# xuanjiangliu/robotic-discovery-platform

Hardware: AMD Instinct MI355X
Metric: U-Net train imgs/sec at 256×256 (1/2/4/8 GPU); e2e frames/sec + p50 latency (higher is better)
Workload: dtype bf16; 1 GPU; model=UNet(3,1) bilinear decoder, 17.26M params, global_batch=64, per_gpu_batch=64, image_size=256, parallelism=dp1, impl=native, optimizer=Adam(lr=1e-4), loss=bce, sync_bn=False, hipgraph=False

## Files before the change

### csrc/bindings.cpp

```cpp
#include <torch/extension.h>
#include <c10/hip/HIPGuard.h>
#include <c10/hip/HIPStream.h>
#include <hip/hip_runtime.h>
#include <dlfcn.h>
#include <link.h>
#include <chrono>
#include <cmath>
#include <climits>
#include <cstdlib>
#include <cstring>
#include <functional>
#include <memory>
#include <vector>
#include <array>

#include "rdp_api.h"

namespace {

hipStream_t cur_stream() { return c10::hip::getCurrentHIPStream().stream(); }

void note_device(int& dev, const torch::Tensor& t) {
  if (!t.defined() || !t.is_cuda()) return;
  const int d = t.get_device();
// ... 461 lines not shown
    if (sp) TORCH_CHECK(rows + conv_stats_rows((long)nn * a1.H * a1.W, Cout, bm_pref) <= avail_rows, "stats slab too small");
    RdpConv c;
    conv_bind(c, kX1, a1, n0, nn);
    conv_bind(c, kX2, a2, n0, nn);
    conv_bind(c, kY1, o1, n0, nn);
    conv_bind(c, kY2, o2, n0, nn);
    conv_weights(c, w);
    c.stats = sp ? sp + (long)rows * 2 * Cout : nullptr;
    c.Cout = Cout;
    c.escale = esc; c.eshift = esh; c.erelu = relu;
    RdpConvFuse fuse;
    if (pool) { fuse.pool = po.image(n0); fuse.ppitch = po.pitch; }
    if (up) {
      fuse.up = uo.image(n0); fuse.upitch = uo.pitch; fuse.uH = uo.H; fuse.uW = uo.W;
      fuse.uoy = up_oy; fuse.uox = up_ox;
    }
    float* const wsp = ws ? ws->data_ptr<float>() : nullptr;
    const long wsn = ws ? (long)ws->numel() : 0L;
    const bool want_fused = pool || up;
    auto pooled = std::make_shared<int>(0);
    const int fmode = wfrag && esc && !sp && !y2 && taps == 9 && !packed && bm_pref == 0
                          ? rdp_conv_rowband_frag_auto(nn, a1.H, a1.W, a1.C, c.C2, Cout) : 0;
    int r = -1;
    if (fmode > 0) {
      RdpConv cf = c;
      cf.w = wfrag->data_ptr(); cf.wbytes = wfrag->numel() * 2; cf.ldw = 0;
      const long pbytes = pool ? po.span_bytes(nn) : 0;
      const int rb = RDP_PLAN(rdp_conv_rowband_ex(cf, fuse.pool, pbytes, fuse.ppitch, fmode, st));
      if (rb >= 0) {
        *pooled = rb == 1 ? 1 : 0;
        r = 0;
      }
    }
    if (r < 0) {
      r = RDP_PLAN(rdp_conv_igemm(c, taps, packed, bm_pref, wsp, wsn, fuse, want_fused ? pooled.get() : nullptr,
                                  RdpConvBnBwd{}, nullptr, st));
    }
    TORCH_CHECK(r >= 0, "conv_fwd: unsupported shape (C1=", a1.C, ", C2=", c.C2, ", Cout=", Cout, ")");
    void* const py1 = c.y1;
    const int oH = o1.H, oW = o1.W, oC = o1.C, op1 = o1.pitch;
    if (pool && !*pooled)
      TORCH_CHECK(RDP_PLAN(rdp_maxpool2_fwd(py1, op1, fuse.pool, fuse.ppitch, nn, oH, oW, oC, st)) == 0,
                  "conv_fwd: maxpool");
    if (up && !*pooled)
      TORCH_CHECK(RDP_PLAN(rdp_upsample2_fwd(py1, op1, fuse.up, fuse.upitch, nn, oH, oW, fuse.uH, fuse.uW, fuse.uoy,
                                             fuse.uox, oC, nullptr, st)) == 0,
                  "conv_fwd: upsample");
    rows += r;
  }
  return rows;
}


int conv_wgrad(torch::Tensor x1, c10::optional<torch::Tensor> x2, torch::Tensor dy, int taps, int packed, int cin_real,
               torch::Tensor slab, torch::Tensor out, int accumulate, int splits, int variant) {
  Act a1 = act(x1, "x1"), a2;
  if (x2) a2 = act(*x2, "x2");
  Act d = act(dy, "dy");
  TORCH_CHECK(d.N == a1.N && d.H == a1.H && d.W == a1.W, "dy spatial mismatch");
  check_f32(slab, "slab");
  check_f32(out, "out");
  const int Cin = packed ? cin_real : a1.C + (x2 ? a2.C : 0);
  TORCH_CHECK(out.numel() == (long)d.C * taps * Cin, "wgrad out numel mismatch");
  const int nc = chunk_images({a1, a2, d}, a1.N);
  int r = 0;
  for (int n0 = 0; n0 < a1.N; n0 += nc) {
    const int nn = std::min(nc, a1.N - n0);
    void* const px1 = a1.image(n0);
    void* const px2 = x2 ? a2.image(n0) : nullptr;
    void* const pdy = d.image(n0);
    const long bx1 = a1.span_bytes(nn), bx2 = x2 ? a2.span_bytes(nn) : 0, bdy = d.span_bytes(nn);
    const int C2 = x2 ? a2.C : 0, p2 = x2 ? a2.pitch : 0, acc = n0 > 0 ? 1 : accumulate;
    float* const slp = slab.data_ptr<float>();
    const long sln = slab.numel();
    float* const outp = out.data_ptr<float>();
    r = RDP_PLAN(rdp_conv_wgrad(px1, px2, bx1, bx2, a1.C, C2, a1.pitch, p2, pdy, bdy, d.pitch, slp, sln, outp, acc, nn,
                                a1.H, a1.W, d.C, taps, packed, cin_real, splits, variant, st));
    TORCH_CHECK(r >= 0, "conv_wgrad: unsupported shape or slab too small (code ", r, ")");
  }
  return r;
}

int wgrad_first_bn(torch::Tensor x, torch::Tensor da, torch::Tensor y, torch::Tensor coef, torch::Tensor coef2,
                   torch::Tensor slab, torch::Tensor out, int cin_real, int accumulate, int splits) {
  Act a = act(x, "x"), d = act(da, "da"), b = act(y, "y");
  TORCH_CHECK(a.C == 8 && d.C == 64 && b.C == 64, "wgrad_first_bn: x must have 8 (packed) and da / y 64 channels");
  TORCH_CHECK(d.N == a.N && d.H == a.H && d.W == a.W && b.N == a.N && b.H == a.H && b.W == a.W,
              "wgrad_first_bn: spatial mismatch");
  check_f32(coef, "coef"); check_f32(coef2, "coef2"); check_f32(slab, "slab"); check_f32(out, "out");
  TORCH_CHECK(coef.numel() >= 4 * 64 && coef2.numel() >= 3 * 64, "wgrad_first_bn: coef / coef2 too small");
  TORCH_CHECK(out.numel() == 64l * 9 * cin_real, "wgrad_first_bn: out numel mismatch");
  if (a.bytes >= (1l << 31) || d.bytes >= (1l << 31) || b.bytes >= (1l << 31)) return -1;
  if (((long)a.N * a.H * a.W) % 64) return -1;
  const int r = RDP_PLAN(rdp_wgrad_first_bn(a.ptr, a.bytes, a.pitch, d.ptr, d.bytes, d.pitch, b.ptr, b.bytes, b.pitch,
                                            coef.data_ptr<float>(), coef2.data_ptr<float>(), slab.data_ptr<float>(),
                                            slab.numel(), out.data_ptr<float>(), accumulate, a.N, a.H, a.W, cin_real,
                                            splits, st));
  TORCH_CHECK(r > 0, "wgrad_first_bn: slab too small (code ", r, ")");
  return r;
}

long wgrad_slab_elems(int N, int H, int W, int Cin, int Cout, int taps, int packed, int splits) {
  return rdp_conv_wgrad_slab_elems(N, H, W, Cin, Cout, taps, packed, splits);
}

void bn_finalize(torch::Tensor stats, int T, long count, torch::Tensor gamma, torch::Tensor beta,
                 c10::optional<torch::Tensor> rmean, c10::optional<torch::Tensor> rvar,
                 c10::optional<torch::Tensor> nbt, double momentum, double eps, torch::Tensor coef,
                 c10::optional<torch::Tensor> ws) {
  const int C = gamma.numel();
  check_f32(stats, "stats"); check_f32(gamma, "gamma"); check_f32(beta, "beta"); check_f32(coef, "coef");
  TORCH_CHECK(stats.numel() >= (long)T * 2 * C && coef.numel() >= 4 * C, "bn_finalize sizes");
  float* rm = nullptr; float* rv = nullptr; long long* nb = nullptr;
  if (rmean) { check_f32(*rmean, "rmean"); rm = rmean->data_ptr<float>(); }
  if (rvar) { check_f32(*rvar, "rvar"); rv = rvar->data_ptr<float>(); }
  if (nbt) { TORCH_CHECK(nbt->scalar_type() == torch::kInt64 && nbt->is_cuda(), "nbt int64"); nb = (long long*)nbt->data_ptr(); }
  RDP_PLAN(rdp_bn_finalize(stats.data_ptr<float>(), T, C, count, gamma.data_ptr<float>(), beta.data_ptr<float>(), rm, rv, nb,
                  (float)momentum, (float)eps, coef.data_ptr<float>(), ws_ptr(ws, 2 * C), st));
}

void bn_eval_coef(torch::Tensor gamma, torch::Tensor beta, torch::Tensor rmean, torch::Tensor rvar, double eps,
                  torch::Tensor coef) {
  const int C = gamma.numel();
  check_f32(coef, "coef");
  RDP_PLAN(rdp_bn_eval_coef(C, gamma.data_ptr<float>(), beta.data_ptr<float>(), rmean.data_ptr<float>(), rvar.data_ptr<float>(),
                   (float)eps, coef.data_ptr<float>(), st));
}

void bn_relu_apply(torch::Tensor y, torch::Tensor out, torch::Tensor coef, int relu) {
  Act a = act(y, "y"), o = act(out, "out");
  TORCH_CHECK(a.N == o.N && a.H == o.H && a.W == o.W && a.C == o.C, "bn_relu_apply shape");
  TORCH_CHECK(coef.numel() >= 4 * a.C, "coef");
  TORCH_CHECK(RDP_PLAN(rdp_bn_relu_apply(a.ptr, a.pitch, o.ptr, o.pitch, coef.data_ptr<float>(), a.N * a.H * a.W, a.C, relu,
                                st)) == 0, "bn_relu_apply");
}

int conv_dgrad_bnred(torch::Tensor dy, torch::Tensor w, torch::Tensor dx, torch::Tensor y_bn, torch::Tensor coef,
                     torch::Tensor partial) {
  Act a = act(dy, "dy"), o = act(dx, "dx"), b = act(y_bn, "y_bn");
  check_w(w);
  TORCH_CHECK(o.N == a.N && o.H == a.H && o.W == a.W && b.N == a.N && b.H == a.H && b.W == a.W && b.C == o.C,
              "conv_dgrad_bnred: shape mismatch");
  TORCH_CHECK(w.size(0) == o.C, "w rows != Cout");
  check_f32(coef, "coef");
  check_f32(partial, "partial");
  TORCH_CHECK(coef.numel() >= 4l * o.C, "coef must hold 4*C floats");
  TORCH_CHECK(partial.numel() >= 1024l * 2 * o.C, "partial too small");
  if (chunk_images({a, o, b}, a.N) < a.N) return -1;
  RdpConv c;
  conv_bind(c, kX1, a, 0, a.N);
  conv_bind(c, kY1, o, 0, a.N);
  conv_weights(c, w);
  c.Cout = o.C;
  c.stats = partial.data_ptr<float>();
  RdpRingFuse f;
  f.bn_y = b.ptr; f.bn_ypitch = b.pitch; f.bn_coef = coef.data_ptr<float>();
  return RDP_PLAN(rdp_conv_ring_ex(c, 256, f, st));
}

int conv_dgrad_splitk_bnred(torch::Tensor dy, torch::Tensor w, torch::Tensor dx, torch::Tensor y_bn,
                            torch::Tensor coef, torch::Tensor partial, c10::optional<torch::Tensor> ws) {
  Act a = act(dy, "dy"), o = act(dx, "dx"), b = act(y_bn, "y_bn");
  check_w(w);
  TORCH_CHECK(o.N == a.N && o.H == a.H && o.W == a.W && b.N == a.N && b.H == a.H && b.W == a.W && b.C == o.C,
              "conv_dgrad_splitk_bnred: shape mismatch");
  TORCH_CHECK(w.size(0) == o.C && w.size(1) >= 9l * a.C, "conv_dgrad_splitk_bnred: w must be [Cout][9 * Cin]");
  check_f32(coef, "coef");
  check_f32(partial, "partial");
  TORCH_CHECK(coef.numel() >= 4l * o.C, "coef must hold 4*C floats");
  TORCH_CHECK(partial.numel() >= 512l * 2 * o.C, "partial too small");
  if (ws) check_f32(*ws, "ws");
  if (chunk_images({a, o, b}, a.N) < a.N) return -1;
  RdpConv c;
  conv_bind(c, kX1, a, 0, a.N);
  conv_bind(c, kY1, o, 0, a.N);
  conv_weights(c, w);
  c.Cout = o.C;
  RdpConvBnBwd bn;
  bn.bny = b.ptr; bn.bnypitch = b.pitch; bn.bncoef = coef.data_ptr<float>(); bn.bnpart = partial.data_ptr<float>();
  float* const wsp = ws ? ws->data_ptr<float>() : nullptr;
// ... 1078 lines not shown
              "u8 / int16 HxW contiguous CPU tensor");
  const int h = img.size(0), w = img.size(1), bpp = (int)img.element_size();
  TORCH_CHECK(h > 0 && w > 0 && level >= 0 && level <= 9 && bands >= 1, "png_encode: bad size / level / bands");
  std::string out((size_t)rdp_png_encode_bound(w, h, bpp, bands), '\0');
  long len;
  {
    py::gil_scoped_release nogil;
    len = rdp_png_encode_gray((const uint8_t*)img.data_ptr(), w, h, bpp, level, bands, (uint8_t*)&out[0],
                              (long)out.size());
  }
  TORCH_CHECK(len > 0, "png encode failed");
  out.resize((size_t)len);
  return py::bytes(out);
}


void preprocess(torch::Tensor bgr, torch::Tensor ystart, torch::Tensor ysize, torch::Tensor yw, torch::Tensor xstart,
                torch::Tensor xsize, torch::Tensor xw, torch::Tensor out, int rgb) {
  TORCH_CHECK(bgr.is_cuda() && bgr.scalar_type() == torch::kUInt8 && bgr.dim() == 3 && bgr.size(2) == 3 &&
              bgr.is_contiguous(), "bgr u8 HxWx3");
  Act o = act(out, "out");
  TORCH_CHECK(o.N == 1 && o.C == 8 && o.pitch == 8, "out must be [1,OH,OW,8] contiguous");
  TORCH_CHECK(ystart.numel() == o.H && xstart.numel() == o.W && yw.numel() == (long)o.H * 16 &&
              xw.numel() == (long)o.W * 16, "aa tables");
  rdp_preprocess(bgr.data_ptr(), bgr.size(0), bgr.size(1), ystart.data_ptr<int>(), ysize.data_ptr<int>(),
                 yw.data_ptr<float>(), xstart.data_ptr<int>(), xsize.data_ptr<int>(), xw.data_ptr<float>(), o.H, o.W,
                 rgb, o.ptr, unplanned_stream());
}

void mask_upsample(torch::Tensor m, torch::Tensor out, torch::Tensor count) {
  TORCH_CHECK(m.is_cuda() && m.scalar_type() == torch::kUInt8 && m.dim() == 2 && m.is_contiguous(), "m");
  TORCH_CHECK(out.is_cuda() && out.scalar_type() == torch::kUInt8 && out.dim() == 2 && out.is_contiguous(), "out");
  TORCH_CHECK(count.is_cuda() && count.scalar_type() == torch::kInt32, "count int32");
  rdp_mask_upsample(m.data_ptr(), m.size(0), m.size(1), out.data_ptr(), out.size(0), out.size(1),
                    (unsigned*)count.data_ptr(), unplanned_stream());
}

}

void register_serve_runtime(py::module_& m);

PYBIND11_MODULE(TORCH_EXTENSION_NAME, m) {
  register_serve_runtime(m);
  m.doc() = "rdp MI355X (gfx950) HIP kernels";
  m.def("stream_wait", &stream_wait, "waiter stream waits for the work issued so far on waitee (recorded in plans)");
  m.def("event_create", &event_create, "runtime-owned cross-stream event (id)");
  m.def("event_record", &event_record, py::arg("id"), py::arg("stream"), "record event id on stream (recorded in plans)");
  m.def("stream_wait_event", &stream_wait_event, py::arg("stream"), py::arg("id"),
        "stream waits for the last record of event id (recorded in plans)");
  m.def("plan_begin", &plan_begin);
  m.def("plan_end", &plan_end);
  m.def("plan_abort", &plan_abort);
  m.def("plan_replay", &plan_replay, py::arg("id"), py::arg("host_call") = py::none());
  m.def("plan_kinds", &plan_kinds);
  m.def("plan_recording", &plan_recording);
  m.def("comm_bind", &comm_bind, "resolve RCCL from the library torch loaded; returns its path");
  m.def("comm_all_reduce", on_device(&comm_all_reduce), py::arg("buf"), py::arg("comm"),
        "in-place SUM all-reduce over an RCCL communicator on the current stream (recorded in plans)");
  m.def("rows_fold", on_device(&rows_fold), py::arg("buf"), py::arg("rows"), py::arg("width"), py::arg("out"));
  m.def("rows_hilo", on_device(&rows_hilo), py::arg("sums"), py::arg("buf"), py::arg("width"));
  m.def("comm_async_error", &comm_async_error, py::arg("comm"), "(code, message) of ncclCommGetAsyncError");
  m.def("comm_abort", &comm_abort, py::arg("comm"), "ncclCommAbort");
  m.def("comm_info", &comm_info, py::arg("comm"), "(ncclCommCount, ncclCommUserRank, ncclCommCuDevice)");
  m.def("comm_emulate", &comm_emulate, py::arg("us"), py::arg("blocks"), py::arg("scratch") = py::none(),
        py::arg("traffic_bytes") = 0, "RDP_DDP_EMULATE: the modelled all-reduce on the current stream (recorded in plans)");
  m.def("plan_mark", &plan_mark, "record a host call point (replay calls host_call(tag) there)");
  m.def("plan_pause", &plan_pause);
  m.def("plan_resume", &plan_resume);
  m.def("plan_size", &plan_size);
  m.def("plan_free", &plan_free);
  m.def("conv_fwd", on_device(&conv_fwd), py::arg("x1"), py::arg("x2"), py::arg("w"), py::arg("taps"), py::arg("packed"),
        py::arg("y1"), py::arg("y2"), py::arg("stats"), py::arg("bm_pref"), py::arg("affine"), py::arg("relu"),
        py::arg("ws") = py::none(), py::arg("pool") = py::none(), py::arg("up") = py::none(),
        py::arg("up_oy") = 0, py::arg("up_ox") = 0, py::arg("wfrag") = py::none());
  m.def("conv_ws_elems", [](int N, int H, int W, int C1, int C2, int Cout, int taps, int packed, int bm_pref) {
    return rdp_conv_ws_elems(N, H, W, C1, C2, Cout, taps, packed, bm_pref);
  });
  m.def("conv_stats_rows", &conv_stats_rows);
  m.def("conv_wgrad", on_device(&conv_wgrad), py::arg("x1"), py::arg("x2"), py::arg("dy"), py::arg("taps"),
        py::arg("packed"), py::arg("cin_real"), py::arg("slab"), py::arg("out"), py::arg("accumulate"),
        py::arg("splits"), py::arg("variant"));
  m.def("conv_fwd_bnin", on_device(&conv_fwd_bnin), py::arg("x_pre"), py::arg("w"), py::arg("y"), py::arg("stats"),
        py::arg("in_coef"), py::arg("a_out") = py::none());
  m.def("wgrad_first_bn", on_device(&wgrad_first_bn));
  m.def("wgrad_slab_elems", &wgrad_slab_elems);
  m.def("wgrad_halo_slab_elems", &rdp_conv_wgrad_halo_slab_elems);
  m.def("bn_finalize", on_device(&bn_finalize));
  m.def("bn_eval_coef", on_device(&bn_eval_coef));
  m.def("bn_relu_apply", on_device(&bn_relu_apply));
  m.def("bn_relu_bwd_reduce", on_device(&bn_relu_bwd_reduce));
  m.def("conv_dgrad_bnred", on_device(&conv_dgrad_bnred));
  m.def("conv_dgrad_splitk_bnred", on_device(&conv_dgrad_splitk_bnred), py::arg("dy"), py::arg("w"), py::arg("dx"),
        py::arg("y_bn"), py::arg("coef"), py::arg("partial"), py::arg("ws") = py::none());
  m.def("bn_bwd_finalize", on_device(&bn_bwd_finalize));
  m.def("bn_relu_bwd_apply", on_device(&bn_relu_bwd_apply));
  m.def("maxpool2_fwd", on_device(&maxpool2_fwd));
  m.def("maxpool2_bwd", on_device(&maxpool2_bwd));
  m.def("bn_relu_apply_pool", on_device(&bn_relu_apply_pool));
  m.def("maxpool2_bwd_bn_reduce", on_device(&maxpool2_bwd_bn_reduce));
  m.def("upsample2_fwd", on_device(&upsample2_fwd), py::arg("x"), py::arg("out"), py::arg("oy"), py::arg("ox"),
        py::arg("coef") = py::none());
  m.def("upT_shuffle", on_device(&upT_shuffle));
  m.def("conv_upT_fwd", on_device(&conv_upT_fwd));
  m.def("conv_upT_dgrad", on_device(&conv_upT_dgrad));
  m.def("conv_wgrad_upT", on_device(&conv_wgrad_upT));
  m.def("upT_unshuffle", on_device(&upT_unshuffle));
  m.def("colsum_bf16", on_device(&colsum_bf16));
  m.def("upsample2_bwd", on_device(&upsample2_bwd), py::arg("dout"), py::arg("dx"), py::arg("oy"), py::arg("ox"),
        py::arg("y") = py::none(), py::arg("coef") = py::none(), py::arg("partial") = py::none());
  m.def("head_partial_blocks", &head_partial_blocks);
  m.def("head_fwd", on_device(&head_fwd), py::arg("a"), py::arg("w"), py::arg("b"), py::arg("target"), py::arg("logits"),
        py::arg("partial"), py::arg("sums"), py::arg("loss"), py::arg("dice_w"), py::arg("dice_eps"),
        py::arg("coef") = py::none(), py::arg("gpart") = py::none(), py::arg("bnpart") = py::none(),
        py::arg("gscale") = 1.0);
  m.def("head_grad_finalize", on_device(&head_grad_finalize));
  m.def("head_bwd", on_device(&head_bwd), py::arg("a"), py::arg("w"), py::arg("logits"), py::arg("target"), py::arg("sums"),
        py::arg("da"), py::arg("partial"), py::arg("gw"), py::arg("gb"), py::arg("dice_w"), py::arg("dice_eps"),
        py::arg("gscale"), py::arg("coef") = py::none(), py::arg("bnpart") = py::none());
  m.def("head_bn_bwd_apply", on_device(&head_bn_bwd_apply));
  m.def("head_mask", on_device(&head_mask));
  m.def("headk_partial_blocks", &headk_partial_blocks);
  m.def("headk_fwd", on_device(&headk_fwd), py::arg("a"), py::arg("w"), py::arg("b"), py::arg("labels"),
        py::arg("logits"), py::arg("partial"), py::arg("sums"), py::arg("loss"), py::arg("class_weights") = py::none(),
        py::arg("dice_w") = 0.0, py::arg("dice_eps") = 1.0);
  m.def("headk_bwd", on_device(&headk_bwd), py::arg("a"), py::arg("w"), py::arg("logits"), py::arg("labels"),
        py::arg("sums"), py::arg("da"), py::arg("partial"), py::arg("gw"), py::arg("gb"), py::arg("gscale") = 1.0,
        py::arg("class_weights") = py::none(), py::arg("dice_w") = 0.0, py::arg("dice_eps") = 1.0);
  m.def("headk_mask", on_device(&headk_mask), py::arg("a"), py::arg("w"), py::arg("b"), py::arg("cls"),
        py::arg("mask"));
  m.def("seg_confusion_blocks", &seg_confusion_blocks);
  m.def("seg_confusion_block_pixels", &seg_confusion_block_pixels);
  m.def("seg_confusion", on_device(&seg_confusion), py::arg("logits"), py::arg("target"), py::arg("K"),
        py::arg("counts"), py::arg("thr") = 0.0, py::arg("max_blocks") = 0);
  m.def("conv_head_mask", on_device(&conv_head_mask));
  m.def("conv_headk_mask", on_device(&conv_headk_mask), py::arg("x"), py::arg("w"), py::arg("coef"), py::arg("head_w"),
        py::arg("head_b"), py::arg("cls"), py::arg("mask"));
  m.def("conv_rowband_chain", on_device(&conv_rowband_chain));
  m.def("conv_rowband", on_device(&conv_rowband));
  m.def("rowband_frag_mode", &rdp_conv_rowband_frag_auto, py::arg("n"), py::arg("h"), py::arg("w"), py::arg("c1"),
        py::arg("c2"), py::arg("cout"));
  m.def("adam", on_device(&adam), py::arg("p"), py::arg("g"), py::arg("m"), py::arg("v"), py::arg("shadow"), py::arg("lr"),
        py::arg("b1"), py::arg("b2"), py::arg("eps"), py::arg("wd"), py::arg("gscale"), py::arg("step"),
        py::arg("inc") = true, py::arg("max_blocks") = 0);
  m.def("grad_sqnorm_blocks", &grad_sqnorm_blocks, py::arg("n"));
  m.def("grad_sqnorm", on_device(&grad_sqnorm), py::arg("g"), py::arg("partial"), py::arg("max_blocks") = 0);
  m.def("optim_ctl", on_device(&optim_ctl), py::arg("partial"), py::arg("nblocks"), py::arg("gscale"), py::arg("clip"),
        py::arg("sched"), py::arg("warmup"), py::arg("total"), py::arg("min_ratio"), py::arg("step"), py::arg("ctl"));
  m.def("adam_ctl", on_device(&adam_ctl), py::arg("p"), py::arg("g"), py::arg("m"), py::arg("v"), py::arg("shadow"),
        py::arg("lr"), py::arg("b1"), py::arg("b2"), py::arg("eps"), py::arg("wd"), py::arg("gscale"), py::arg("step"),
        py::arg("ctl"), py::arg("inc") = true, py::arg("max_blocks") = 0);
  m.def("cast_bf16", on_device(&cast_bf16));
  m.def("h2d_copy", &h2d_copy, py::arg("src"), py::arg("dst"));
  m.def("wprep", on_device(&wprep), py::arg("master"), py::arg("out"), py::arg("segs"), py::arg("nseg"),
        py::arg("step") = py::none(), py::arg("blocks") = 0);
  m.def("wseg_size", &rdp_wseg_size);
  m.def("parcur", &parcur);
  m.def("batch_preprocess", on_device(&batch_preprocess));
  m.def("geo_frames_batch", on_device(&geo_frames_batch));
  m.def("geo_edges", on_device(&geo_edges), py::arg("mask"), py::arg("depth"), py::arg("fx"), py::arg("fy"), py::arg("cx"),
        py::arg("cy"), py::arg("scale"), py::arg("work_i"), py::arg("work_d"), py::arg("pts"), py::arg("npts"),
        py::arg("out"), py::arg("kout"), py::arg("nbins"), py::arg("top"), py::arg("min_points"),
        py::arg("edges") = py::none(), py::arg("hdr") = py::none(), py::arg("m256") = py::none(),
        py::arg("cov") = py::none(), py::arg("sorted") = py::none(), py::arg("gperm") = py::none(),
        py::arg("mask_host") = py::none());
  m.def("geo_nblocks", &geo_nblocks);
  m.def("geo_spline", on_device(&geo_spline), py::arg("out"), py::arg("kout"), py::arg("npts"), py::arg("sorted"),
        py::arg("gperm"), py::arg("u"), py::arg("res"), py::arg("s"), py::arg("k"), py::arg("nsamp"), py::arg("eps"),
// ... 28 lines not shown
```

### csrc/conv_wgrad.hip

```cpp
#include "common.h"
#include "rdp_api.h"
#include <algorithm>
#include <stdlib.h>
#include <string.h>

struct WgradArgs {
  const u16* x1;
  const u16* x2;
  uint32_t xbytes1, xbytes2;
  int C1, C2, pitch1, pitch2;
  const u16* dy;
  uint32_t dybytes;
  int dypitch;
  float* slab;
  int H, W, M, Cout, Cin;
  int taps, packed;
  int ncols, ncols_pad;
  int colTiles, coutTiles, splits;
  int pix_per_split;
  uint32_t fw_m, fw_s, fh_m, fh_s;
  int uH2 = 0, uW2 = 0, uoy = 0, uox = 0;
};

RDP_DEV int swz(int p) { return (((p >> 1) & 1) << 1) | (((p >> 3) & 1) << 2); }
// ... 650 lines not shown
      else hipLaunchKernelGGL((conv_wgrad_halo_kernel<64, false>), dim3(nblk), dim3(256), 0, s, h);
    }
    rdp_wgrad_reduce(slab, out, h.splits, Cout, h.ncols, 9, a.Cin, a.Cin, accumulate, s);
    return h.splits;
  }
  a.colTiles = (a.ncols + 255) / 256;
  a.ncols_pad = a.colTiles * 256;
  a.coutTiles = Cout / 64;
  if (splits < 1) splits = 1;
  int pps = (a.M + splits - 1) / splits;
  pps = (pps + 63) / 64 * 64;
  a.pix_per_split = pps;
  a.splits = (a.M + pps - 1) / pps;
  if ((long)a.splits * Cout * a.ncols_pad > slab_elems) return -2;
  if ((long)a.splits * Cout * a.ncols_pad * 4l >= (1l << 31)) return -3;
  FastDiv fw = make_fastdiv(W), fh = make_fastdiv(H);
  a.fw_m = fw.m; a.fw_s = fw.s; a.fh_m = fh.m; a.fh_s = fh.s;
  const int nblk = a.colTiles * a.coutTiles * a.splits;
  if (packed) hipLaunchKernelGGL((conv_wgrad_kernel<true>), dim3(nblk), dim3(512), 0, s, a);
  else hipLaunchKernelGGL((conv_wgrad_kernel<false>), dim3(nblk), dim3(512), 0, s, a);
  rdp_wgrad_reduce(slab, out, a.splits, Cout, a.ncols_pad, taps, packed ? 8 : a.Cin, packed ? cin_real : a.Cin,
                   accumulate, s);
  return a.splits;
}

extern "C" int rdp_conv_wgrad_upT(const void* du, long dubytes, int C, int dupitch, int H2, int W2, int oy, int ox,
                                  const void* x, long xbytes, int Cin, int xpitch, int N, int h, int w, float* slab,
                                  long slab_elems, float* out, int accumulate, int splits, hipStream_t s) {
  if (C % 64 || Cin % 64 || oy < 0 || ox < 0 || 2 * h + oy > H2 || 2 * w + ox > W2) return -1;
  if (dubytes >= (1l << 31) || xbytes >= (1l << 31)) return -1;
  WgradArgs a;
  a.x1 = (const u16*)du; a.x2 = nullptr; a.xbytes1 = (uint32_t)dubytes; a.xbytes2 = 0;
  a.C1 = C; a.C2 = 0; a.pitch1 = dupitch; a.pitch2 = dupitch;
  a.dy = (const u16*)x; a.dybytes = (uint32_t)xbytes; a.dypitch = xpitch;
  a.slab = slab; a.H = h; a.W = w; a.M = N * h * w; a.Cout = Cin;
  a.taps = 4; a.packed = 0; a.Cin = C; a.ncols = 4 * C;
  a.uH2 = H2; a.uW2 = W2; a.uoy = oy; a.uox = ox;
  a.colTiles = (a.ncols + 255) / 256;
  a.ncols_pad = a.colTiles * 256;
  a.coutTiles = Cin / 64;
  if (splits < 1) splits = 1;
  int pps = (a.M + splits - 1) / splits;
  pps = (pps + 63) / 64 * 64;
  a.pix_per_split = pps;
  a.splits = (a.M + pps - 1) / pps;
  if ((long)a.splits * a.Cout * a.ncols_pad > slab_elems) return -2;
  if ((long)a.splits * a.Cout * a.ncols_pad * 4l >= (1l << 31)) return -3;
  FastDiv fw = make_fastdiv(w), fh = make_fastdiv(h);
  a.fw_m = fw.m; a.fw_s = fw.s; a.fh_m = fh.m; a.fh_s = fh.s;
  const int nblk = a.colTiles * a.coutTiles * a.splits;
  hipLaunchKernelGGL((conv_wgrad_kernel<false, true>), dim3(nblk), dim3(512), 0, s, a);
  rdp_wgrad_reduce(slab, out, a.splits, Cin, a.ncols_pad, 4, C, C, accumulate, s);
  return a.splits;
}

struct FirstWgradArgs {
  const u16* x;
  uint32_t xbytes;
  int xpitch;
  const u16* da;
  uint32_t dabytes;
  int dapitch;
  const u16* y;
  uint32_t ybytes;
  int ypitch;
  const float* coef;
  const float* coef2;
  float* slab;
  uint32_t slab_bytes;
  int H, W, M, pix_per_split;
  uint32_t fw_m, fw_s, fh_m, fh_s;
};
constexpr int FWG_NCOLS = 80;

RDP_DEV void fw_unpack8(const uint4& v, float* f) {
  const uint32_t w[4] = {v.x, v.y, v.z, v.w};
#pragma unroll
  for (int i = 0; i < 4; ++i) {
    f[2 * i] = __uint_as_float(w[i] << 16);
    f[2 * i + 1] = __uint_as_float(w[i] & 0xffff0000u);
  }
}

__global__ __launch_bounds__(256, 2) void wgrad_first_bn_kernel(const FirstWgradArgs a) {
  constexpr int SUB = 64 * 128;
  constexpr int BUF = 3 * SUB;
  __shared__ __attribute__((aligned(16))) char smem[2 * BUF];
  const int lane = threadIdx.x & 63;
  const int wave = __builtin_amdgcn_readfirstlane(threadIdx.x >> 6);
  const int split = (int)xcd_remap(blockIdx.x, gridDim.x);
  const int pbeg = split * a.pix_per_split;
  const int nks = max(0, min(a.M, pbeg + a.pix_per_split) - pbeg) / 64;
  const auto rx = make_rsrc(a.x, a.xbytes);
  const auto rda = make_rsrc(a.da, a.dabytes);
  const auto ry = make_rsrc(a.y, a.ybytes);

  const int tc = threadIdx.x & 7, tr0 = threadIdx.x >> 3;
  float ss[8], hh[8], cA[8], cB[8], cK[8];
#pragma unroll
  for (int k = 0; k < 8; ++k) {
    const int c = 8 * tc + k;
    ss[k] = a.coef[128 + c]; hh[k] = a.coef[192 + c];
    cA[k] = a.coef2[c]; cB[k] = a.coef2[64 + c]; cK[k] = a.coef2[128 + c];
  }
  uint4 vd[2], vy[2];
  auto load_dz = [&](int ks) {
#pragma unroll
    for (int u = 0; u < 2; ++u) {
      const int m = pbeg + ks * 64 + tr0 + 32 * u;
      vd[u] = bload16(rda, (uint32_t)(m * a.dapitch + 8 * tc) * 2u);
      vy[u] = bload16(ry, (uint32_t)(m * a.ypitch + 8 * tc) * 2u);
    }
  };
  auto store_dz = [&](char* buf) {
#pragma unroll
    for (int u = 0; u < 2; ++u) {
      const int p = tr0 + 32 * u;
      float fd[8], fy[8];
      fw_unpack8(vd[u], fd);
      fw_unpack8(vy[u], fy);
      uint32_t o[4];
#pragma unroll
      for (int k = 0; k < 8; k += 2) {
        const float g0 = fmaf(fy[k], ss[k], hh[k]) > 0.f ? fd[k] : 0.f;
        const float g1 = fmaf(fy[k + 1], ss[k + 1], hh[k + 1]) > 0.f ? fd[k + 1] : 0.f;
        o[k / 2] = pack2bf(fmaf(cA[k], g0, fmaf(cB[k], fy[k], cK[k])),
                           fmaf(cA[k + 1], g1, fmaf(cB[k + 1], fy[k + 1], cK[k + 1])));
      }
      *(uint4*)(buf + 2 * SUB + p * 128 + 16 * (tc ^ swz(p))) = make_uint4(o[0], o[1], o[2], o[3]);
    }
  };
  const int rowl = lane >> 3, cpos = lane & 7;
  auto issue_x = [&](int ks, char* buf) {
#pragma unroll
    for (int t = 0; t < 4; ++t) {
      const int s = wave * 4 + t, sub = s >> 3, pj = s & 7;
      const int p = pj * 8 + rowl;
      const int g = cpos ^ swz(p);
      const int m = pbeg + ks * 64 + p;
      const uint32_t q = fdiv2((uint32_t)m, a.fw_m, a.fw_s);
      const int w = m - (int)q * a.W;
      const int h = (int)q - (int)fdiv2(q, a.fh_m, a.fh_s) * a.H;
      const int tap = sub * 8 + g;
      const int dr = tap / 3 - 1, ds = tap % 3 - 1;
      const bool ok = (tap < 9) & inb(h + dr, a.H) & inb(w + ds, a.W);
      const uint32_t off = ok ? (uint32_t)((m + dr * a.W + ds) * a.xpitch) * 2u : RDP_OOB;
      dma16_async(rx, (lds_void*)(buf + sub * SUB + pj * 1024), off);
    }
  };

  f32x4 acc[5];
#pragma unroll
  for (int i = 0; i < 5; ++i) acc[i] = f32x4{0.f, 0.f, 0.f, 0.f};
  const int tg = lane >> 4, tq = (lane >> 2) & 3, tpp = lane & 3;
  typedef __attribute__((address_space(3))) bf16x4 lds_v4;

  if (nks > 0) {
    load_dz(0);
    issue_x(0, smem);
    store_dz(smem);
  }
  for (int ks = 0; ks < nks; ++ks) {
    asm volatile("s_waitcnt vmcnt(0) lgkmcnt(0)" ::: "memory");
    raw_barrier();
    const char* cur = smem + (ks & 1) * BUF;
    char* nxt = smem + ((ks + 1) & 1) * BUF;
    const bool more = ks + 1 < nks;
    if (more) {
      load_dz(ks + 1);
      issue_x(ks + 1, nxt);
    }
#pragma unroll
    for (int hf = 0; hf < 2; ++hf) {
      const int p0 = 32 * hf + 8 * tg + tq;
      const int sw0 = swz(p0), sw1 = swz(p0 + 4);
      const int ro0 = p0 * 128 + 8 * (tpp & 1), ro1 = ro0 + 4 * 128;
      auto frag = [&](const char* base, int i) {
        const int c = 2 * i + (tpp >> 1);
        const bf16x4 b0 = __builtin_amdgcn_ds_read_tr16_b64_v4i16((lds_v4*)(base + ro0 + 16 * (c ^ sw0)));
        const bf16x4 b1 = __builtin_amdgcn_ds_read_tr16_b64_v4i16((lds_v4*)(base + ro1 + 16 * (c ^ sw1)));
        return __builtin_shufflevector(b0, b1, 0, 1, 2, 3, 4, 5, 6, 7);
      };
      const bf16x8 fb = frag(cur + 2 * SUB, wave);
      bf16x8 fa[5];
#pragma unroll
      for (int i = 0; i < 4; ++i) fa[i] = frag(cur, i);
      fa[4] = frag(cur + SUB, 0);
#pragma unroll
      for (int i = 0; i < 5; ++i) acc[i] = __builtin_amdgcn_mfma_f32_16x16x32_bf16(fa[i], fb, acc[i], 0, 0, 0);
    }
    if (more) store_dz(nxt);
  }

  const auto rs = make_rsrc(a.slab, a.slab_bytes);
  const int co = 16 * wave + (lane & 15);
#pragma unroll
  for (int i = 0; i < 5; ++i) {
    const int col = 16 * i + 4 * (lane >> 4);
    const uint32_t off = (uint32_t)(((long)split * 64 + co) * FWG_NCOLS + col) * 4u;
    uint4 v;
    v.x = __float_as_uint(acc[i][0]); v.y = __float_as_uint(acc[i][1]);
    v.z = __float_as_uint(acc[i][2]); v.w = __float_as_uint(acc[i][3]);
    bstore16(rs, off, v);
  }
}

extern "C" int rdp_wgrad_first_bn(const void* x, long xbytes, int xpitch, const void* da, long dabytes, int dapitch,
                                  const void* y, long ybytes, int ypitch, const float* coef, const float* coef2,
                                  float* slab, long slab_elems, float* out, int accumulate, int N, int H, int W,
                                  int cin_real, int splits, hipStream_t s) {
  const long M = (long)N * H * W;
  if (M % 64 || cin_real > 8 || cin_real < 1) return -1;
  if (xbytes >= (1l << 31) || dabytes >= (1l << 31) || ybytes >= (1l << 31)) return -1;
  if (xpitch % 8 || dapitch % 8 || ypitch % 8) return -1;
  splits = (int)std::max(1L, std::min<long>(splits, M / 64));
  long pps = (M + splits - 1) / splits;
  pps = (pps + 63) / 64 * 64;
  splits = (int)((M + pps - 1) / pps);
  const long per_split = 64l * FWG_NCOLS;
  if ((long)splits * per_split > slab_elems) return -2;
  if ((long)splits * per_split * 4l >= (1l << 31)) return -3;
  FirstWgradArgs a;
  a.x = (const u16*)x; a.xbytes = (uint32_t)xbytes; a.xpitch = xpitch;
  a.da = (const u16*)da; a.dabytes = (uint32_t)dabytes; a.dapitch = dapitch;
  a.y = (const u16*)y; a.ybytes = (uint32_t)ybytes; a.ypitch = ypitch;
  a.coef = coef; a.coef2 = coef2;
  a.slab = slab; a.slab_bytes = (uint32_t)(splits * per_split * 4l);
  a.H = H; a.W = W; a.M = (int)M; a.pix_per_split = (int)pps;
  FastDiv fw = make_fastdiv(W), fh = make_fastdiv(H);
  a.fw_m = fw.m; a.fw_s = fw.s; a.fh_m = fh.m; a.fh_s = fh.s;
  hipLaunchKernelGGL(wgrad_first_bn_kernel, dim3(splits), dim3(256), 0, s, a);
  rdp_wgrad_reduce(slab, out, splits, 64, FWG_NCOLS, 9, 8, cin_real, accumulate, s);
  return splits;
}

extern "C" long rdp_conv_wgrad_slab_elems(int N, int H, int W, int Cin, int Cout, int taps, int packed, int splits) {
  const int ncols = packed ? 72 : taps * Cin;
  const int ncols_pad = (ncols + 255) / 256 * 256;
  const long M = (long)N * H * W;
  long pps = (M + splits - 1) / splits;
  pps = (pps + 63) / 64 * 64;
  const long sp = (M + pps - 1) / pps;
  return sp * Cout * ncols_pad;
}

extern "C" long rdp_conv_wgrad_halo_slab_elems(int N, int H, int W, int Cin, int Cout) {
  const long M = (long)N * H * W;
  const bool halo = Cin % 64 == 0 && Cout % 64 == 0 && (W % 64 == 0 || (W >= 32 && 64 % W == 0 && (H * W) % 64 == 0));
  if (!halo) return 0;
  const int BN = Cout % 128 == 0 ? 128 : 64;
  const long tiles = (long)(Cin / 64) * (Cout / BN);
  const long target = BN == 64 ? 512 : 256;
  long hsp = std::max<long>(1, (target + tiles - 1) / tiles);
  hsp = std::min<long>(hsp, std::max<long>(1, M / 64));
  return hsp * Cout * 9L * Cin;
}
```

### csrc/rdp_api.h

```cpp
#pragma once
#include <hip/hip_runtime_api.h>

#include "rdp_host_api.h"

struct RdpConv {
  const void* x1 = nullptr;
  const void* x2 = nullptr;
  long xbytes1 = 0, xbytes2 = 0;
  int C1 = 0, C2 = 0, pitch1 = 0, pitch2 = 0;
  const void* w = nullptr;
  long wbytes = 0;
  int ldw = 0;
  void* y1 = nullptr;
  void* y2 = nullptr;
  long ybytes1 = 0, ybytes2 = 0;
  int Cy1 = 0, ypitch1 = 0, ypitch2 = 0;
  float* stats = nullptr;
  int N = 0, H = 0, W = 0, Cout = 0;
  const float* escale = nullptr;
  const float* eshift = nullptr;
  int erelu = 0;
};
struct RdpConvFuse {
  void* pool = nullptr;
  int ppitch = 0;
  void* up = nullptr;
  int upitch = 0, uH = 0, uW = 0, uoy = 0, uox = 0;
};
struct RdpConvBnBwd {
  const void* bny = nullptr;
  int bnypitch = 0;
  const float* bncoef = nullptr;
  float* bnpart = nullptr;
};
struct RdpRingFuse {
  const void* bn_y = nullptr;
  int bn_ypitch = 0;
  const float* bn_coef = nullptr;
  const float* iscale = nullptr;
  const float* ishift = nullptr;
  void* aout = nullptr;
  long abytes = 0;
  int apitch = 0;
};

extern "C" {

int rdp_comm_emulate(double us, int blocks, hipStream_t s);
int rdp_comm_emulate_traffic(double us, int blocks, void* scratch, long scratch_bytes, long traffic_bytes,
                             hipStream_t s);

int rdp_conv_first(const RdpConv& c, hipStream_t s);

int rdp_conv_halo_tiles(int N, int H, int W, int C1, int C2, int Cout, int taps, int packed);
int rdp_conv_halo(const RdpConv& c, hipStream_t s);

int rdp_conv_upT_fwd(const void* x, long xbytes, int Cin, int pitch, const void* w, long wbytes, int ldw, void* u,
                     long ubytes, int upitch, const float* bias, int N, int h, int wd, int H2, int W2, int oy,
                     int ox, int C, hipStream_t s);
int rdp_conv_upT_dgrad(const void* du, long dubytes, int C, int dupitch, int H2, int W2, int oy, int ox,
                       const void* wd, long wbytes, int ldw, void* dx, long dxbytes, int Cin, int dxpitch, int N,
                       int h, int wdt, hipStream_t s);
int rdp_conv_igemm(const RdpConv& c, int taps, int packed, int bm_pref, float* ws, long ws_elems,
                   const RdpConvFuse& fuse, int* pooled, const RdpConvBnBwd& bn, int* bnrows, hipStream_t s);
long rdp_conv_ws_elems(int N, int H, int W, int C1, int C2, int Cout, int taps, int packed, int bm_pref);

int rdp_conv_ring(const RdpConv& c, int max_blocks, hipStream_t s);
int rdp_conv_ring_ex(const RdpConv& c, int max_blocks, const RdpRingFuse& f, hipStream_t s);
int rdp_conv_ring_head(const void* x, long xbytes, int C, int pitch, const void* w, long wbytes, int ldw, int Cout,
                       int N, int H, int W, const float* escale, const float* eshift, const float* hw,
                       const float* hb, float hthr, void* mask, hipStream_t s);
int rdp_conv_ring_headk(const void* x, long xbytes, int C, int pitch, const void* w, long wbytes, int ldw, int Cout,
                        int N, int H, int W, const float* escale, const float* eshift, const float* hw,
                        const float* hb, int K, int cls, void* mask, hipStream_t s);
int rdp_conv_ring_pool(const RdpConv& c, void* pool, int ppitch, hipStream_t s);
int rdp_conv_ring2(const RdpConv& c, int max_blocks, int cout_total, int co0, hipStream_t s);

long rdp_conv_rowband_bytes(int N, int H, int W, int Cin, int Cout, int pool);
int rdp_conv_rowband_frag_auto(int N, int H, int W, int C1, int C2, int Cout);
int rdp_conv_rowband(const RdpConv& c, void* pool, long pbytes, int ppitch, hipStream_t s);
int rdp_conv_rowband_ex(const RdpConv& c, void* pool, long pbytes, int ppitch, int wfrag, hipStream_t s);
int rdp_conv_rowband_chain(int nl, const void* x, long xbytes, int C0, int xpitch, const void* const* w,
                           const long* wbytes, const int* ldw, void* const* y, const long* ybytes,
                           const int* ypitch, const int* cout, const float* const* escale,
                           const float* const* eshift, int N, int H, int W, int* cnt, int* err, hipStream_t s);

void rdp_wgrad_reduce(float* slab, float* out, int splits, int Cout, int ncols_pad, int taps, int cin_pad,
                      int cin_real, int accumulate, hipStream_t s);
int rdp_conv_wgrad(const void* x1, const void* x2, long xbytes1, long xbytes2, int C1, int C2, int pitch1,
                   int pitch2, const void* dy, long dybytes, int dypitch, float* slab, long slab_elems, float* out,
                   int accumulate, int N, int H, int W, int Cout, int taps, int packed, int cin_real, int splits,
                   int variant, hipStream_t s);
int rdp_conv_wgrad_upT(const void* du, long dubytes, int C, int dupitch, int H2, int W2, int oy, int ox,
                       const void* x, long xbytes, int Cin, int xpitch, int N, int h, int w, float* slab,
                       long slab_elems, float* out, int accumulate, int splits, hipStream_t s);
int rdp_wgrad_first_bn(const void* x, long xbytes, int xpitch, const void* da, long dabytes, int dapitch,
                       const void* y, long ybytes, int ypitch, const float* coef, const float* coef2, float* slab,
                       long slab_elems, float* out, int accumulate, int N, int H, int W, int cin_real, int splits,
                       hipStream_t s);
long rdp_conv_wgrad_slab_elems(int N, int H, int W, int Cin, int Cout, int taps, int packed, int splits);
long rdp_conv_wgrad_halo_slab_elems(int N, int H, int W, int Cin, int Cout);

int rdp_batch_augment(const void* x, const void* y, const int* idx, const float* params, int S, int N, int H, int W,
                      void* x_out, float* tgt_f, void* tgt_u, hipStream_t s);
int rdp_area_maxtap();
int rdp_resize_area_u8(const void* in, int h, int w, int C, const int* ys, const int* yn, const double* yw,
                       const int* xs, const int* xn, const double* xw, int H, int W, int swap_rb, void* out,
                       hipStream_t s);

int rdp_geo_spline_res_len(int nsamp);
int rdp_geo_spline_batch(int n, int nbins, int kcap, const int* const* kout, const int* const* npts,
                         double* const* sorted, double* const* u, int ecap, double s, int k, int nsamp, double eps,
                         int min_points, int min_edge, const int* const* cov, int ncov, double* const* res,
                         const void* const* mask, void* const* mask_host, long mask_bytes, hipStream_t st);
int rdp_geo_spline(const double* out, int nbins, int kcap, const int* kout, const int* npts, double* sorted,
                   int* gperm, double* u, int ecap, double s, int k, int nsamp, double eps, int min_points,
                   int min_edge, const int* cov, int ncov, double* res, double* dbg, int presorted,
                   const void* mask, void* mask_host, long mask_bytes, hipStream_t st);

int rdp_geo_nblocks(int H);
long rdp_geo_work_ints(int H, int W);
int rdp_geo_edges(const void* mask, const void* depth, int H, int W, double fx, double fy, double cx, double cy,
                  double scale, int* counts, double* xmin, double* xmax, double* pts, int cap, int* npts,
                  double* out, int kcap, int* kout, int nbins, double top, int min_points, double* edges, int ecap,
                  int* hdr, const void* m256, int mh, int mw, int* cov, double* sorted, int* gperm, int secap,
                  void* mask_host, hipStream_t s);
int rdp_geo_edges_batch(int n, const void* const* mask, const void* const* depth, int H, int W, double fx,
                        double fy, double cx, double cy, double scale, int* const* counts, double* const* xmin,
                        double* const* xmax, double* const* pts, int cap, int* const* npts, double* const* out,
                        int kcap, int* const* kout, int nbins, double top, int min_points, const void* const* m256,
                        int mh, int mw, int* const* cov, double* const* sorted, int* const* gperm, int secap,
                        void* const* mask_host, hipStream_t s);

int rdp_head_partial_blocks(long M);
int rdp_head_fwd(const void* a, int apitch, const float* w, const float* b, const float* target, float* logits,
                 float* partial, float* sums, float* loss, int M, float dice_w, float dice_eps, const float* coef,
                 float* gpart, float* bnpart, float gscale, hipStream_t s);
int rdp_head_grad_finalize(const float* gpart, int M, float* gw, float* gb, hipStream_t s);
int rdp_head_bwd(const void* a, int apitch, const float* w, const float* logits, const float* target,
                 const float* sums, void* da, int dapitch, float* partial, float* gw, float* gb, int M,
                 float dice_w, float dice_eps, float gscale, const float* coef, float* bnpart, hipStream_t s);
int rdp_head_bn_bwd_apply(const void* y, int ypitch, const float* w, const float* logits, const float* target,
                          const float* sums, const float* coef, const float* coef2, void* dy, int dypitch, int M,
                          float dice_w, float dice_eps, float gscale, hipStream_t s);
int rdp_head_mask(const void* a, int apitch, const float* w, const float* b, float logit_thr, void* mask, int M,
                  hipStream_t s);

int rdp_headk_partial_blocks(long M);
int rdp_headk_fwd(const void* a, int apitch, const float* w, const float* b, const void* labels, float* logits,
                  float* partial, float* sums, float* loss, int M, int K, const float* cw, float dice_w,
                  float dice_eps, hipStream_t s);
int rdp_headk_bwd(const void* a, int apitch, const float* w, const float* logits, const void* labels,
                  const float* sums, void* da, int dapitch, float* partial, float* gw, float* gb, int M, int K,
                  float gscale, const float* cw, float dice_w, float dice_eps, hipStream_t s);
int rdp_headk_mask(const void* a, int apitch, const float* w, const float* b, int cls, void* mask, int M, int K,
                   hipStream_t s);

int rdp_jpeg_entropy_gpu(const void* scan, long cap_bytes, const int* nbits, const void* tables, const int* geo,
                         void* coefs, long cap_coefs, int* work, long work_words, int* status, int S,
                         long* stats_word, hipStream_t st);

int rdp_bn_finalize(const float* stats, int T, int C, long count, const float* gamma, const float* beta,
                    float* rmean, float* rvar, long long* nbt, float momentum, float eps, float* coef, float* ws,
                    hipStream_t s);
int rdp_rows_fold(const float* buf, int T, int K, double* out, hipStream_t s);
int rdp_rows_hilo(const double* in, float* buf, int K, hipStream_t s);
int rdp_bn_eval_coef(int C, const float* gamma, const float* beta, const float* rmean, const float* rvar, float eps,
                     float* coef, hipStream_t s);
int rdp_bn_relu_apply(const void* y, int ypitch, void* out, int opitch, const float* coef, int M, int C, int relu,
                      hipStream_t s);
int rdp_bn_relu_bwd_reduce(const void* da, int dapitch, const void* y, int ypitch, const float* coef, int M, int C,
                           int relu, float* partial, int max_blocks, hipStream_t s);
int rdp_bn_bwd_finalize(const float* partial, int T, int C, long count, const float* gamma, const float* coef,
                        float* dgamma, float* dbeta, float* coef2, float* ws, hipStream_t s);
int rdp_bn_relu_bwd_apply(const void* da, int dapitch, const void* y, int ypitch, const float* coef,
                          const float* coef2, void* dy, int dypitch, int M, int C, int relu, hipStream_t s);

int rdp_adam(float* p, const void* g, int g_bf16, float* m, float* v, void* shadow, long n, float lr, float b1,
             float b2, float eps, float wd, float gscale, int* step, int inc, int max_blocks, hipStream_t s);
int rdp_adam_ctl(float* p, const void* g, int g_bf16, float* m, float* v, void* shadow, long n, float lr, float b1,
                 float b2, float eps, float wd, float gscale, int* step, const float* ctl, int inc, int max_blocks,
                 hipStream_t s);
// ... 52 lines not shown
```

Before: 3367 images/s.

## Add three-stage software pipeline to first-layer BN-fused weight-gradient kernel

Templates the first-layer wgrad kernel on a stage count and makes a 3-stage pipeline the default. The x-tile async DMA buffers are split from the dz buffer, and dz register loads are kept R steps ahead, so global loads overlap more MFMA work. The original 2-stage path stays selectable with stages=1. This adds shared memory (kept within two blocks per CU) and register pressure from the extra vd/vy sets, and it relies on a hand-tuned vmcnt wait count.

```diff
diff --git a/csrc/bindings.cpp b/csrc/bindings.cpp
--- a/csrc/bindings.cpp
+++ b/csrc/bindings.cpp
@@ -567,7 +567,7 @@
 }
 
 int wgrad_first_bn(torch::Tensor x, torch::Tensor da, torch::Tensor y, torch::Tensor coef, torch::Tensor coef2,
-                   torch::Tensor slab, torch::Tensor out, int cin_real, int accumulate, int splits) {
+                   torch::Tensor slab, torch::Tensor out, int cin_real, int accumulate, int splits, int stages) {
   Act a = act(x, "x"), d = act(da, "da"), b = act(y, "y");
   TORCH_CHECK(a.C == 8 && d.C == 64 && b.C == 64, "wgrad_first_bn: x must have 8 (packed) and da / y 64 channels");
   TORCH_CHECK(d.N == a.N && d.H == a.H && d.W == a.W && b.N == a.N && b.H == a.H && b.W == a.W,
@@ -577,10 +577,11 @@
   TORCH_CHECK(out.numel() == 64l * 9 * cin_real, "wgrad_first_bn: out numel mismatch");
   if (a.bytes >= (1l << 31) || d.bytes >= (1l << 31) || b.bytes >= (1l << 31)) return -1;
   if (((long)a.N * a.H * a.W) % 64) return -1;
+  TORCH_CHECK(stages == 0 || stages == 1 || stages == 3, "wgrad_first_bn: stages must be 0 (default), 1 or 3");
   const int r = RDP_PLAN(rdp_wgrad_first_bn(a.ptr, a.bytes, a.pitch, d.ptr, d.bytes, d.pitch, b.ptr, b.bytes, b.pitch,
                                             coef.data_ptr<float>(), coef2.data_ptr<float>(), slab.data_ptr<float>(),
                                             slab.numel(), out.data_ptr<float>(), accumulate, a.N, a.H, a.W, cin_real,
-                                            splits, st));
+                                            splits, stages, st));
   TORCH_CHECK(r > 0, "wgrad_first_bn: slab too small (code ", r, ")");
   return r;
 }
@@ -1825,7 +1826,9 @@
         py::arg("splits"), py::arg("variant"));
   m.def("conv_fwd_bnin", on_device(&conv_fwd_bnin), py::arg("x_pre"), py::arg("w"), py::arg("y"), py::arg("stats"),
         py::arg("in_coef"), py::arg("a_out") = py::none());
-  m.def("wgrad_first_bn", on_device(&wgrad_first_bn));
+  m.def("wgrad_first_bn", on_device(&wgrad_first_bn), py::arg("x"), py::arg("da"), py::arg("y"), py::arg("coef"),
+        py::arg("coef2"), py::arg("slab"), py::arg("out"), py::arg("cin_real"), py::arg("accumulate"),
+        py::arg("splits"), py::arg("stages") = 0);
   m.def("wgrad_slab_elems", &wgrad_slab_elems);
   m.def("wgrad_halo_slab_elems", &rdp_conv_wgrad_halo_slab_elems);
   m.def("bn_finalize", on_device(&bn_finalize));
diff --git a/csrc/conv_wgrad.hip b/csrc/conv_wgrad.hip
--- a/csrc/conv_wgrad.hip
+++ b/csrc/conv_wgrad.hip
@@ -756,10 +756,15 @@
   }
 }
 
+template <int STAGES>
 __global__ __launch_bounds__(256, 2) void wgrad_first_bn_kernel(const FirstWgradArgs a) {
   constexpr int SUB = 64 * 128;
-  constexpr int BUF = 3 * SUB;
-  __shared__ __attribute__((aligned(16))) char smem[2 * BUF];
+  constexpr int XBUF = 2 * SUB;
+  constexpr int NX = STAGES == 1 ? 2 : STAGES;
+  constexpr int R = STAGES == 1 ? 1 : STAGES - 1;
+  static_assert(NX * XBUF + 2 * SUB <= 80 * 1024, "two blocks per CU");
+  __shared__ __attribute__((aligned(16))) char smem[NX * XBUF + 2 * SUB];
+  char* const dzs = smem + NX * XBUF;
   const int lane = threadIdx.x & 63;
   const int wave = __builtin_amdgcn_readfirstlane(threadIdx.x >> 6);
   const int split = (int)xcd_remap(blockIdx.x, gridDim.x);
@@ -777,22 +782,23 @@
     ss[k] = a.coef[128 + c]; hh[k] = a.coef[192 + c];
     cA[k] = a.coef2[c]; cB[k] = a.coef2[64 + c]; cK[k] = a.coef2[128 + c];
   }
-  uint4 vd[2], vy[2];
-  auto load_dz = [&](int ks) {
+  uint4 vd[R][2], vy[R][2];
+  auto load_dz = [&](int ks, int set) {
+    const bool live = ks < nks;
 #pragma unroll
     for (int u = 0; u < 2; ++u) {
       const int m = pbeg + ks * 64 + tr0 + 32 * u;
-      vd[u] = bload16(rda, (uint32_t)(m * a.dapitch + 8 * tc) * 2u);
-      vy[u] = bload16(ry, (uint32_t)(m * a.ypitch + 8 * tc) * 2u);
+      vd[set][u] = bload16(rda, live ? (uint32_t)(m * a.dapitch + 8 * tc) * 2u : RDP_OOB);
+      vy[set][u] = bload16(ry, live ? (uint32_t)(m * a.ypitch + 8 * tc) * 2u : RDP_OOB);
     }
   };
-  auto store_dz = [&](char* buf) {
+  auto store_dz = [&](int set, char* dzb) {
 #pragma unroll
     for (int u = 0; u < 2; ++u) {
       const int p = tr0 + 32 * u;
       float fd[8], fy[8];
-      fw_unpack8(vd[u], fd);
-      fw_unpack8(vy[u], fy);
+      fw_unpack8(vd[set][u], fd);
+      fw_unpack8(vy[set][u], fy);
       uint32_t o[4];
 #pragma unroll
       for (int k = 0; k < 8; k += 2) {
@@ -801,11 +807,12 @@
         o[k / 2] = pack2bf(fmaf(cA[k], g0, fmaf(cB[k], fy[k], cK[k])),
                            fmaf(cA[k + 1], g1, fmaf(cB[k + 1], fy[k + 1], cK[k + 1])));
       }
-      *(uint4*)(buf + 2 * SUB + p * 128 + 16 * (tc ^ swz(p))) = make_uint4(o[0], o[1], o[2], o[3]);
+      *(uint4*)(dzb + p * 128 + 16 * (tc ^ swz(p))) = make_uint4(o[0], o[1], o[2], o[3]);
     }
   };
   const int rowl = lane >> 3, cpos = lane & 7;
   auto issue_x = [&](int ks, char* buf) {
+    const bool live = ks < nks;
 #pragma unroll
     for (int t = 0; t < 4; ++t) {
       const int s = wave * 4 + t, sub = s >> 3, pj = s & 7;
@@ -817,7 +824,7 @@
       const int h = (int)q - (int)fdiv2(q, a.fh_m, a.fh_s) * a.H;
       const int tap = sub * 8 + g;
       const int dr = tap / 3 - 1, ds = tap % 3 - 1;
-      const bool ok = (tap < 9) & inb(h + dr, a.H) & inb(w + ds, a.W);
+      const bool ok = live & (tap < 9) & inb(h + dr, a.H) & inb(w + ds, a.W);
       const uint32_t off = ok ? (uint32_t)((m + dr * a.W + ds) * a.xpitch) * 2u : RDP_OOB;
       dma16_async(rx, (lds_void*)(buf + sub * SUB + pj * 1024), off);
     }
@@ -828,22 +835,7 @@
   for (int i = 0; i < 5; ++i) acc[i] = f32x4{0.f, 0.f, 0.f, 0.f};
   const int tg = lane >> 4, tq = (lane >> 2) & 3, tpp = lane & 3;
   typedef __attribute__((address_space(3))) bf16x4 lds_v4;
-
-  if (nks > 0) {
-    load_dz(0);
-    issue_x(0, smem);
-    store_dz(smem);
-  }
-  for (int ks = 0; ks < nks; ++ks) {
-    asm volatile("s_waitcnt vmcnt(0) lgkmcnt(0)" ::: "memory");
-    raw_barrier();
-    const char* cur = smem + (ks & 1) * BUF;
-    char* nxt = smem + ((ks + 1) & 1) * BUF;
-    const bool more = ks + 1 < nks;
-    if (more) {
-      load_dz(ks + 1);
-      issue_x(ks + 1, nxt);
-    }
+  auto mfma_step = [&](const char* xb, const char* dzb) {
 #pragma unroll
     for (int hf = 0; hf < 2; ++hf) {
       const int p0 = 32 * hf + 8 * tg + tq;
@@ -855,15 +847,69 @@
         const bf16x4 b1 = __builtin_amdgcn_ds_read_tr16_b64_v4i16((lds_v4*)(base + ro1 + 16 * (c ^ sw1)));
         return __builtin_shufflevector(b0, b1, 0, 1, 2, 3, 4, 5, 6, 7);
       };
-      const bf16x8 fb = frag(cur + 2 * SUB, wave);
+      const bf16x8 fb = frag(dzb, wave);
       bf16x8 fa[5];
 #pragma unroll
-      for (int i = 0; i < 4; ++i) fa[i] = frag(cur, i);
-      fa[4] = frag(cur + SUB, 0);
+      for (int i = 0; i < 4; ++i) fa[i] = frag(xb, i);
+      fa[4] = frag(xb + SUB, 0);
 #pragma unroll
       for (int i = 0; i < 5; ++i) acc[i] = __builtin_amdgcn_mfma_f32_16x16x32_bf16(fa[i], fb, acc[i], 0, 0, 0);
     }
-    if (more) store_dz(nxt);
+  };
+
+  if constexpr (STAGES == 1) {
+    if (nks > 0) {
+      load_dz(0, 0);
+      issue_x(0, smem);
+      store_dz(0, dzs);
+    }
+    for (int ks = 0; ks < nks; ++ks) {
+      asm volatile("s_waitcnt vmcnt(0) lgkmcnt(0)" ::: "memory");
+      raw_barrier();
+      const int cb = ks & 1;
+      const bool more = ks + 1 < nks;
+      if (more) {
+        load_dz(ks + 1, 0);
+        issue_x(ks + 1, smem + (cb ^ 1) * XBUF);
+      }
+      mfma_step(smem + cb * XBUF, dzs + cb * SUB);
+      if (more) store_dz(0, dzs + (cb ^ 1) * SUB);
+    }
+  } else {
+#pragma unroll
+    for (int j = 0; j < R; ++j) {
+      load_dz(j, j);
+      if (j + 1 < R) issue_x(j, smem + j * XBUF);
+    }
+    store_dz(0, dzs);
+    issue_x(R - 1, smem + (R - 1) * XBUF);
+    int slot = 0;
+    auto step = [&](int ks, int j) {
+      asm volatile("s_waitcnt vmcnt(%0) lgkmcnt(0)" ::"n"(8 * (STAGES - 2)) : "memory");
+      raw_barrier();
+      load_dz(ks + R, j);
+      __builtin_amdgcn_sched_barrier(0);
+      mfma_step(smem + slot * XBUF, dzs + (ks & 1) * SUB);
+      __builtin_amdgcn_sched_barrier(0);
+      store_dz((j + 1) % R, dzs + ((ks + 1) & 1) * SUB);
+      const int last = slot == 0 ? NX - 1 : slot - 1;
+      issue_x(ks + R, smem + last * XBUF);
+      slot = slot + 1 == NX ? 0 : slot + 1;
+    };
+    int k0 = 0;
+    for (; k0 + R <= nks; k0 += R) {
+#pragma unroll
+      for (int j = 0; j < R; ++j) step(k0 + j, j);
+    }
+#pragma unroll
+    for (int j = 0; j + 1 < R; ++j)
+      if (k0 + j < nks) step(k0 + j, j);
+#pragma unroll
+    for (int r = 0; r < R; ++r)
+#pragma unroll
+      for (int u = 0; u < 2; ++u)
+        asm volatile("" ::"v"(vd[r][u].x), "v"(vd[r][u].y), "v"(vd[r][u].z), "v"(vd[r][u].w), "v"(vy[r][u].x),
+                     "v"(vy[r][u].y), "v"(vy[r][u].z), "v"(vy[r][u].w));
   }
 
   const auto rs = make_rsrc(a.slab, a.slab_bytes);
@@ -882,9 +928,10 @@
 extern "C" int rdp_wgrad_first_bn(const void* x, long xbytes, int xpitch, const void* da, long dabytes, int dapitch,
                                   const void* y, long ybytes, int ypitch, const float* coef, const float* coef2,
                                   float* slab, long slab_elems, float* out, int accumulate, int N, int H, int W,
-                                  int cin_real, int splits, hipStream_t s) {
+                                  int cin_real, int splits, int stages, hipStream_t s) {
   const long M = (long)N * H * W;
   if (M % 64 || cin_real > 8 || cin_real < 1) return -1;
+  if (stages != 0 && stages != 1 && stages != 3) return -1;
   if (xbytes >= (1l << 31) || dabytes >= (1l << 31) || ybytes >= (1l << 31)) return -1;
   if (xpitch % 8 || dapitch % 8 || ypitch % 8) return -1;
   splits = (int)std::max(1L, std::min<long>(splits, M / 64));
@@ -903,7 +950,8 @@
   a.H = H; a.W = W; a.M = (int)M; a.pix_per_split = (int)pps;
   FastDiv fw = make_fastdiv(W), fh = make_fastdiv(H);
   a.fw_m = fw.m; a.fw_s = fw.s; a.fh_m = fh.m; a.fh_s = fh.s;
-  hipLaunchKernelGGL(wgrad_first_bn_kernel, dim3(splits), dim3(256), 0, s, a);
+  if (stages == 1) hipLaunchKernelGGL(wgrad_first_bn_kernel<1>, dim3(splits), dim3(256), 0, s, a);
+  else hipLaunchKernelGGL(wgrad_first_bn_kernel<3>, dim3(splits), dim3(256), 0, s, a);
   rdp_wgrad_reduce(slab, out, splits, 64, FWG_NCOLS, 9, 8, cin_real, accumulate, s);
   return splits;
 }
diff --git a/csrc/rdp_api.h b/csrc/rdp_api.h
--- a/csrc/rdp_api.h
+++ b/csrc/rdp_api.h
@@ -97,7 +97,7 @@
 int rdp_wgrad_first_bn(const void* x, long xbytes, int xpitch, const void* da, long dabytes, int dapitch,
                        const void* y, long ybytes, int ypitch, const float* coef, const float* coef2, float* slab,
                        long slab_elems, float* out, int accumulate, int N, int H, int W, int cin_real, int splits,
-                       hipStream_t s);
+                       int stages, hipStream_t s);
 long rdp_conv_wgrad_slab_elems(int N, int H, int W, int Cin, int Cout, int taps, int packed, int splits);
 long rdp_conv_wgrad_halo_slab_elems(int N, int H, int W, int Cin, int Cout);
 
```

New measurement: 3371 images/s, median of 5. Within noise of the previous version (+0.1%).
